# mpasha3/trips-py

Hardware: AMD Instinct MI355X
Metric: krylov_iters_per_sec (higher is better)
Workload: dtype f32

## Files before the change

### include/trk.h

```cpp
#ifndef TRK_H
#define TRK_H

#include <stdint.h>

#ifdef __cplusplus
extern "C" {
#endif

#define TRK_OK 0
#define TRK_EINVAL (-1)
#define TRK_EHIP (-2)
#define TRK_ENOMEM (-3)
#define TRK_EUNSUPPORTED (-4)
#define TRK_ENCCL (-5)

#define TRK_SQRT_NUM 1
#define TRK_SQRT_DEN 2

typedef struct trk_op trk_op;
typedef void* trk_stream;
typedef struct trk_comm trk_comm;

int trk_version(void);
const char* trk_last_error(void);
// ... 171 lines not shown
                                  double beta0, double m_eff, double x1, double x2, double xatol, int maxfun);
int trk_host_worker_post_hess_fixed(trk_host_worker* w, const double* H, int64_t h_row_stride, int64_t h_col_stride, int k,
                                    double beta0, double lam);
int trk_host_worker_post_hess_dp(trk_host_worker* w, const double* H, int64_t h_row_stride, int64_t h_col_stride, int k,
                                 double beta0, const double* bproj, double target, double extra);
int trk_host_worker_collect_vec(trk_host_worker* w, double* lam_out, int* have_out, double* y, int k, double* resid_out);

int trk_cgls_iterate(trk_op* A, int k_first, int n_iters, float* p, float* r, float* t, float* w, float* X, int64_t x_ld,
                     int keep_history, const float* x_prev, const float* x_true, double* S, double* NP,
                     int np_capacity_blocks, int* n_np_inout, double* PG, double* PD, int pcap, int grouping,
                     trk_stream stream);
int trk_cgls_iterate_fused(trk_op* A, int k_first, int n_iters, float* P, int64_t p_ld, float* R, int64_t r_ld, float* t,
                           float* w, float* X, int64_t x_ld, int keep_history, const float* x_prev, const float* x_true,
                           double* S, double* PG, double* PD, int pcap, double* NP, int np_capacity_blocks,
                           int* n_g_inout, int* n_np_inout, trk_stream stream);

int trk_finalize_batched(const double* partials, int nblocks, int nvals, int batches, double* out, int out_stride,
                         trk_stream stream);

int trk_gemv_t(const float* V, int64_t ld, int k, int64_t n, const float* r, const float* w2, double* h_dev,
               trk_stream stream);
int trk_gemv_nt(const float* V, int64_t ld, int k, int64_t n, const double* h_dev, const float* w_in, float* w_out,
                double* g_dev, trk_stream stream);
int trk_gemv_t_x(const float* V, int64_t ld, int k, int64_t n, const float* r, const float* xrow, double* h, double* h_x,
                 trk_stream stream);
int trk_gemv_t2(const float* V, int64_t ld, int k, int64_t n, const float* r, const float* r2, double* h2k_dev,
                trk_stream stream);
int trk_cgs_coeffs(double* G_dev, int ldg, const double* h_dev, const double* g_new_dev, int k, int passes, double* c_dev,
                   trk_stream stream);
int trk_cgs_coeffs_rho(double* G_dev, int ldg, const double* h_dev, const double* g_new_dev, int k, int passes, double* c_dev,
// ... 83 lines not shown
```

### trips_py_amd/_lib.py

```python
import ctypes
import os
import shutil
import subprocess
import sys
from concurrent.futures import ThreadPoolExecutor

HERE = os.path.dirname(os.path.abspath(__file__))
CSRC = os.path.join(HERE, "csrc")
INCLUDE = os.path.join(os.path.dirname(HERE), "include")
LIB_PATH = os.path.join(CSRC, "libtrk.so")
SOURCES = ["core.hip", "vecops.hip", "blur2d.hip", "tvops.hip", "radon2d.hip", "spmv.hip", "fanbeam2d.hip", "projected.hip", "cgls_loop.hip", "comm.hip", "cgls_tiled.hip", "cgls_sharded.hip", "ref64.hip"]
HIPCC_FLAGS = ["-O3", "--offload-arch=gfx950", "-std=c++17", "-fPIC", "-I" + INCLUDE, "-I" + CSRC]


class TrkError(RuntimeError):
    pass


def _hipcc():
    exe = shutil.which("hipcc") or "/opt/rocm/bin/hipcc"
    if not os.path.exists(exe):
        raise TrkError("hipcc not found: cannot build libtrk.so (ROCm toolchain required)")
    return exe

# ... 173 lines not shown
                                   ctypes.POINTER(c_int), ctypes.POINTER(c_dbl)]),
    "trk_host_gcv_bidiag": (c_int, [c_f64p, c_f64p, c_int, c_dbl, c_dbl, c_dbl, c_dbl, c_dbl, c_int, ctypes.POINTER(c_dbl),
                                    ctypes.POINTER(c_dbl), ctypes.POINTER(c_int)]),
    "trk_cgls_iterate": (c_int, [c_op, c_int, c_int, c_f32p, c_f32p, c_f32p, c_f32p, c_f32p, c_i64, c_int, c_f32p, c_f32p,
                                 c_f64p, c_f64p, c_int, ctypes.POINTER(c_int), c_f64p, c_f64p, c_int, c_int, c_stream]),
    "trk_cgls_update_xr_src": (c_int, [c_i64, c_i64, c_f64p, c_int, c_f64p, c_int, c_f32p, c_f32p, c_f32p, c_f32p, c_f32p,
                                       c_f32p, c_f64p, c_f64p, c_int, ctypes.POINTER(c_int), c_stream]),
    "trk_cgls_update_grouping": (c_int, [c_i64]),
    "trk_cgls_r_update": (c_int, [c_i64, c_f64p, c_f64p, c_int, c_f32p, c_f32p, c_f64p, c_stream]),
    "trk_cgls_xp_update": (c_int, [c_i64, c_f64p, c_f64p, c_f64p, c_int, c_f32p, c_f32p, c_f32p, c_f32p, c_f32p, c_f64p, c_f64p,
                                   c_int, ctypes.POINTER(c_int), c_stream]),
    "trk_cgls_p_update": (c_int, [c_i64, c_f32p, c_f32p, c_f64p, c_int, c_f64p, c_f64p, c_stream]),
    "trk_cgls_iterate_fused": (c_int, [c_op, c_int, c_int, c_f32p, c_i64, c_f32p, c_i64, c_f32p, c_f32p, c_f32p, c_i64, c_int,
                                       c_f32p, c_f32p, c_f64p, c_f64p, c_f64p, c_int, c_f64p, c_int, ctypes.POINTER(c_int),
                                       ctypes.POINTER(c_int), c_stream]),
    "trk_cgls_tiled_caps": (c_int, [c_op, c_int, c_int, ctypes.POINTER(c_int)]),
    "trk_cgls_iterate_tiled": (c_int, [c_op, c_int, c_int, c_f32p, c_i64, c_f32p, c_i64, c_f32p, c_f32p, c_i64, c_int,
                                       c_f32p, c_f32p, c_f64p, c_f64p, c_f64p, c_int, c_f64p, c_int, ctypes.POINTER(c_int),
                                       ctypes.POINTER(c_int), c_stream]),
    "trk_cgls_iterate_tiled2": (c_int, [c_op, c_int, c_int, c_f32p, c_f32p, c_f32p, c_i64, c_f32p, c_f32p, c_i64, c_int,
                                        c_f32p, c_f32p, c_f64p, c_f64p, c_f64p, c_int, c_f64p, c_int, ctypes.POINTER(c_int),
                                        ctypes.POINTER(c_int), c_stream]),
    "trk_gemv_t": (c_int, [c_f32p, c_i64, c_int, c_i64, c_f32p, c_f32p, c_f64p, c_stream]),
    "trk_gemv_t_x": (c_int, [c_f32p, c_i64, c_int, c_i64, c_f32p, c_f32p, c_f64p, c_f64p, c_stream]),
    "trk_gemv_t2": (c_int, [c_f32p, c_i64, c_int, c_i64, c_f32p, c_f32p, c_f64p, c_stream]),
    "trk_gemv_tn": (c_int, [c_f32p, c_i64, c_int, c_i64, ctypes.POINTER(ctypes.c_void_p), c_int, c_f64p, c_stream]),
    "trk_gram_row_from_sweep": (c_int, [c_f64p, c_int, c_int, c_f64p, c_f64p, c_f64p, c_f64p, c_f64p, c_f64p, c_stream]),
    "trk_gram_tikhonov": (c_int, [c_f64p, c_int, c_f64p, c_int, c_f64p, c_int, c_dbl, c_f64p, c_int, c_int, c_f64p, c_stream]),
    "trk_hess_tikhonov": (c_int, [c_f64p, c_int, c_f64p, c_f64p, c_int, c_f64p, c_f64p, c_f64p, c_dbl, c_int, c_dbl, c_int, c_f64p,
                                  c_stream]),
# ... 113 lines not shown
```

### trips_py_amd/csrc/blur2d.hip

```cpp
#include "trk_internal.h"
#include <hip/hip_ext.h>

#include <cmath>
#include <cstdlib>
#include <type_traits>
#include <vector>

using namespace trk;

namespace {

constexpr int NT = 256;
constexpr int TW = 128;
constexpr int TH = 32;

typedef float f4 __attribute__((ext_vector_type(4)));

__host__ __device__ constexpr int rup4(int v) { return (v + 3) & ~3; }

__device__ __forceinline__ int reflect(int i, int n) {
  if ((unsigned)i < (unsigned)n) return i;
  const int p = 2 * n;
  i %= p;
  if (i < 0) i += p;
// ... 510 lines not shown
  if (trk_timer* t = op->timer)
    if ((op->timer_which == 2 || op->timer_which == tr) && t->used < t->cap) {
      ev0 = t->ev[2 * t->used];
      ev1 = t->ev[2 * t->used + 1];
      ++t->used;
    }
  switch (im->kh) {
    case 3: return launch_slide<3, 6>(im, tr, x1, 0, y, 0, 1, partials, spans_x, nbands, rpb, s, ev0, ev1, fzp);
    case 5: return launch_slide<5, 5>(im, tr, x1, 0, y, 0, 1, partials, spans_x, nbands, rpb, s, ev0, ev1, fzp);
    case 7: return launch_slide<7, 7>(im, tr, x1, 0, y, 0, 1, partials, spans_x, nbands, rpb, s, ev0, ev1, fzp);
    default:
      return launch_slide<9, 9>(im, tr, x1, 0, y, 0, 1, partials, spans_x, nbands, rpb, s, ev0, ev1, fzp);
  }
}

int blur_apply(trk_op* op, int tr, const float* x, int64_t ldx, float* y, int64_t ldy, int batch, double* sumsq,
               hipStream_t s) {
  auto* im = static_cast<BlurImpl*>(op->impl);
  double* part = nullptr;
  int nblk;
  const bool slide_ok = slide_shape_ok(im) && aligned16(x) && aligned16(y) &&
                        (batch == 1 || ((ldx & 3) == 0 && (ldy & 3) == 0));
  if (slide_ok) {
    int spans_x, nbands, rpb;
    const int Usel = (im->kh == 9) ? 9 : (im->kh == 7) ? 7 : (im->kh == 5) ? 5 : 6;
    slide_grid(im->nx, im->ny, batch, im->kh, Usel, &spans_x, &nbands, &rpb);
    nblk = spans_x * nbands;
    if (sumsq)
      if (int rc = scratch_doubles(s, (size_t)nblk * batch, &part)) return rc;
    hipEvent_t ev0 = nullptr, ev1 = nullptr;
// ... 171 lines not shown
    rc = upload(sf, &im->sep_dev[0]);
    if (!rc) rc = upload(st, &im->sep_dev[1]);
  }
  if (rc) {
    trk_op tmp{1, 0, 0, im, nullptr, nullptr, nullptr, 0};
    blur_destroy(&tmp);
    return rc;
  }
  const int64_t n = (int64_t)nx * ny;
  auto* op = new trk_op{1, n, n, im, blur_apply, blur_destroy, nullptr, 0};
  if (slide_shape_ok(im)) op->apply_fused = blur_apply_fused;
  if (slide_shape_ok(im)) op->apply_axpby_plain = blur_apply_axpby_plain;
  *out = op;
  return TRK_OK;
}
```

### trips_py_amd/csrc/cgls_loop.hip

```cpp
#include "trk_internal.h"

using namespace trk;

extern "C" {

int trk_cgls_update_grouping(int64_t n) {
  static const int env = getenv("TRK_CGLS_XP") ? atoi(getenv("TRK_CGLS_XP")) : -1;
  if (env >= 0) return env != 0;
  return n >= ((int64_t)8 << 20) ? 1 : 0;
}

int trk_cgls_iterate(trk_op* A, int k_first, int n_iters, float* p, float* r, float* t, float* w, float* X, int64_t x_ld,
                     int keep_history, const float* x_prev, const float* x_true, double* S, double* NP,
                     int np_capacity_blocks, int* n_np_inout, double* PG, double* PD, int pcap, int grouping,
                     trk_stream stream) {
  TRK_REQUIRE(A && p && r && t && w && X && x_prev && S && NP && n_np_inout, "trk_cgls_iterate: NULL argument");
  TRK_REQUIRE(k_first >= 1 && n_iters >= 0, "trk_cgls_iterate: need k_first >= 1, n_iters >= 0");
  const int64_t m = A->rows, n = A->cols;
  int n_np = *n_np_inout;
  const bool raw = PG && PD && pcap > 0 && A->apply_fused;
  const bool xp_form = (grouping < 0 ? trk_cgls_update_grouping(n) : grouping) == 1;
  for (int k = k_first; k < k_first + n_iters; ++k) {
    double* row = S + 5 * (int64_t)k;
    double *delta = row, *gamma = row + 1;
// ... 61 lines not shown
    if (rc) return rc;
    float* x_new = X + (int64_t)(keep_history ? (k - 1) : ((k - 1) & 1)) * x_ld;
    double* gpub = (k == 1) ? S : S + b - 4;
    rc = trk_cgls_x_update(n, PG, n_g, PD, n_d, x_prev, p_new, x_new, x_true, S + b, gpub,
                           NP + 3 * (int64_t)n_np * (k - 1), np_capacity_blocks, &n_np, stream);
    if (rc) return rc;
    rc = trk_op_apply_fused(A, 1, r_old, w, -1.0, gpub, 1, S + b, 1, r_new, t, PG, pcap, &n_g, stream);
    if (rc) return rc;
    x_prev = x_new;
  }
  *n_g_inout = n_g;
  *n_np_inout = n_np;
  return TRK_OK;
}

}
```

### trips_py_amd/csrc/trk_internal.h

```cpp
#pragma once
#include <hip/hip_runtime.h>
#include <stdint.h>
#include <stddef.h>
#include "trk.h"

namespace trk {

void set_error(const char* fmt, ...) __attribute__((format(printf, 1, 2)));
int fail(int code, const char* fmt, ...) __attribute__((format(printf, 2, 3)));

#define TRK_HIP(expr)                                                                         \
  do {                                                                                        \
    hipError_t e_ = (expr);                                                                   \
    if (e_ != hipSuccess) return ::trk::fail(TRK_EHIP, "%s -> %s (%s:%d)", #expr,             \
                                             hipGetErrorString(e_), __FILE__, __LINE__);      \
  } while (0)

#define TRK_REQUIRE(cond, ...)                                  \
  do {                                                          \
    if (!(cond)) return ::trk::fail(TRK_EINVAL, __VA_ARGS__);   \
  } while (0)

#define TRK_LAUNCH_CHECK() TRK_HIP(hipGetLastError())

// ... 220 lines not shown
  if (i + 256 < s.n) a4 += s.p[i + 256];
  if (i + 320 < s.n) a5 += s.p[i + 320];
  if (i + 384 < s.n) a6 += s.p[i + 384];
  double v = ((a0 + a1) + (a2 + a3)) + ((a4 + a5) + (a6 + a7));
  v = wave_sum(v);
  return __hiloint2double(__builtin_amdgcn_readfirstlane(__double2hiint(v)), __builtin_amdgcn_readfirstlane(__double2loint(v)));
}

inline int ceil_div(int64_t a, int64_t b) { return (int)((a + b - 1) / b); }

inline int stream_nontemporal(int64_t n) {
  static const int env = getenv("TRK_NT") ? atoi(getenv("TRK_NT")) : -1;
  static const int rev = (getenv("TRK_REV") && atoi(getenv("TRK_REV"))) ? 256 : 0;
  if (env >= 0) return env | rev;
  if (n >= kNontemporalLoadsMinFloats) return 51 | 192 | rev;
  return (n >= kNontemporalMinFloats ? (3 | 192) : 0) | rev;
}

inline bool aligned16(const void* p) { return (reinterpret_cast<uintptr_t>(p) & 15u) == 0; }

}

struct trk_timer {
  hipEvent_t* ev;
  int cap, used;
};

namespace trk {
struct TimerScope {
  trk_timer* t;
  hipStream_t s;
// ... 103 lines not shown
```

### trips_py_amd/engine.py

```python
import ctypes

import numpy as np
import torch

from . import _lib

SQRT_NUM = 1
SQRT_DEN = 2


class Coef:

    __slots__ = ("c", "num", "den", "flags", "_keep")

    def __init__(self, c=1.0, num=None, den=None, sqrt_num=False, sqrt_den=False):
        self.c = float(c)
        self.num = _ptr(num)
        self.den = _ptr(den)
        self.flags = (SQRT_NUM if sqrt_num else 0) | (SQRT_DEN if sqrt_den else 0)
        self._keep = (num, den)


_raw_stream = getattr(torch._C, "_cuda_getCurrentRawStream", None)
if _raw_stream is None:
# ... 439 lines not shown
                                       ctypes.byref(c), _ptr(PG), _ptr(PD), int(pcap), int(grouping), self.stream())
        _lib.check(rc, "trk_cgls_iterate")
        return c.value

    def cgls_iterate_fused(self, handle, k_first, n_iters, P, R, t, w, X, keep, x_prev, x_true, S, PG, PD, pcap, NP, np_cap,
                           n_g, n_np):
        cg, cn = ctypes.c_int(int(n_g)), ctypes.c_int(int(n_np))
        rc = self.lib.trk_cgls_iterate_fused(handle, int(k_first), int(n_iters), P.data_ptr(), P.stride(0), R.data_ptr(),
                                             R.stride(0), t.data_ptr(), w.data_ptr(), X.data_ptr(), X.stride(0),
                                             int(bool(keep)), x_prev.data_ptr(), None if x_true is None else x_true.data_ptr(),
                                             _ptr(S), _ptr(PG), _ptr(PD), int(pcap), _ptr(NP), int(np_cap), ctypes.byref(cg),
                                             ctypes.byref(cn), self.stream())
        _lib.check(rc, "trk_cgls_iterate_fused")
        return cg.value, cn.value

    def cgls_tiled_caps(self, handle, np_cap, pcap):
        can = ctypes.c_int(0)
        _lib.check(self.lib.trk_cgls_tiled_caps(handle, int(np_cap), int(pcap), ctypes.byref(can)), "trk_cgls_tiled_caps")
        return bool(can.value)

    def cgls_iterate_tiled(self, handle, k_first, n_iters, P, R, t, X, keep, x_prev, x_true, S, PG, PD, pcap, NP, np_cap,
                           n_g, n_np):
        cg, cn = ctypes.c_int(int(n_g)), ctypes.c_int(int(n_np))
        rc = self.lib.trk_cgls_iterate_tiled(handle, int(k_first), int(n_iters), P.data_ptr(), P.stride(0), R.data_ptr(),
                                             R.stride(0), t.data_ptr(), X.data_ptr(), X.stride(0), int(bool(keep)),
                                             x_prev.data_ptr(), None if x_true is None else x_true.data_ptr(), _ptr(S),
                                             _ptr(PG), _ptr(PD), int(pcap), _ptr(NP), int(np_cap), ctypes.byref(cg),
                                             ctypes.byref(cn), self.stream())
        _lib.check(rc, "trk_cgls_iterate_tiled")
        return cg.value, cn.value
# ... 237 lines not shown
```

### trips_py_amd/solvers/CGLS.py

```python
import numpy as np

from .._io import Formatter, History, as_operator
from ..engine import Coef


class _ShiftedRows:

    def __init__(self, t, shift):
        self.t, self.shift = t, int(shift)

    def data_ptr(self):
        return self.t.data_ptr() + self.shift * self.t.stride(0) * self.t.element_size()

    def stride(self, dim):
        return self.t.stride(dim)

    def row(self, j):
        return self.t[j + self.shift]


def _row_of(X, j, keep):
    if isinstance(X, _ShiftedRows):
        return X.row(j)
    return X[j] if keep else X[j & 1]
# ... 221 lines not shown
            rows = Sh[5:5 * (k + 1)].reshape(k, 5).copy()
            rows[:, 2:5] = Nh[:3 * k].reshape(k, 3)
            rows[k - 1, 1] = Nh[3 * k]
            self._rows = (k, Sh[0], rows)
        return self._rows[1], self._rows[2]

    def row(self, k):
        return self.rows()[1][k - 1]


class CGLSRunFused(CGLSRun):

    PCAP = 4096
    AUTO_MIN_N = 3 * 2 ** 20
    AUTO_MAX_N = 7 * 2 ** 20

    @classmethod
    def auto(cls, n):
        return cls.AUTO_MIN_N <= n <= cls.AUTO_MAX_N

    @staticmethod
    def usable(A, eng):
        return (getattr(eng, "is_native", False) and eng.world == 1 and hasattr(A, "_h") and A.shape[0] == A.shape[1]
                and eng.op_can_fuse(A._h) == 1)

    TILED_MAX_N = 1 << 20
    TILED_DEFAULT = 2

    @classmethod
    def tiled_usable(cls, A, eng):
        return (cls.usable(A, eng) and hasattr(eng, "cgls_tiled_caps") and A.shape[1] <= cls.TILED_MAX_N
                and eng.cgls_tiled_caps(A._h, 1024, cls.PCAP))

    def __init__(self, A, b, x0, max_iter, x_true=None, history=True, tiled=False):
        self.A = A = as_operator(A)
        self.eng = eng = A.engine
        m, n = A.shape
        self.tiled = int(tiled)
        self.max_iter = max_iter = int(max_iter)
        self.bv = eng.to_vec(b, m)
        self.xt = None if x_true is None else eng.to_vec(x_true, n)
        x_start = eng.to_vec(x0, n)
        self.hist = History(eng, history, max_iter, n, "CGLS xHistory")
        self.keep = self.hist.keeps_any
        self.X = self.hist.X
        self.R = eng.empty_basis(2, m)
        self.P = eng.empty_basis(2, n)
        if self.tiled != 2:
            self.P.zero_()
        self.t, self.w = eng.empty(n), eng.empty(m)
        self.S = S = eng.scalars(5 * (max_iter + 1))
        uninit = getattr(eng, "scalars_uninit", eng.scalars)
        self.PG = uninit(self.PCAP)
        self.PD = uninit(self.PCAP)
        self.NP = uninit(3 * 1024 * max_iter)
        self.dist = False
        self.k = 0
        self.n_g = self.n_np = 0
        A.apply(x_start, out=self.w)
        self.n_g = eng.op_apply_fused(A._h, True, self.bv, self.w, -1.0, None, 0, None, 0, self.R[0], self.t,
                                      self.PG.ref(0), self.PCAP)
        self.x_cur = x_start
        self._final = False

    def _step(self):
        eng, A, S = self.eng, self.A, self.S
        if self.tiled:
            x_new = self.hist.row(self.k)
            keep = self.hist.mode == "device"
            X = self.X if self.hist.mode != "stream" else _ShiftedRows(self.X, self.hist.slot(self.k) - self.k)
            self._tiled_call(self.k + 1, 1, X, keep or self.hist.mode == "stream")
            self.k += 1
            self.x_cur = x_new
            return
        self.k += 1
        k = self.k
        b = 5 * k
        p_old, p_new = self.P[(k - 1) & 1], self.P[k & 1]
        r_old, r_new = self.R[(k - 1) & 1], self.R[k & 1]
        gprev = S.ref(0) if k <= 2 else S.ref(5 * (k - 2) + 1)
        n_d = eng.op_apply_fused(A._h, False, self.t, p_old, 0.0 if k == 1 else 1.0, self.PG.ref(0), self.n_g, gprev, 1,
                                 p_new, self.w, self.PD.ref(0), self.PCAP)
        x_new = self.hist.row(k - 1)
        gpub = S.ref(0) if k == 1 else S.ref(b - 4)
        self.n_np = eng.cgls_x_update(self.PG.ref(0), self.n_g, self.PD.ref(0), n_d, self.x_cur, p_new, x_new, self.xt,
                                      S.ref(b), gpub, self.NP.ref(3 * self.n_np * (k - 1)), 1024)
        self.n_g = eng.op_apply_fused(A._h, True, r_old, self.w, -1.0, gpub, 1, S.ref(b), 1, r_new, self.t,
                                      self.PG.ref(0), self.PCAP)
        self.x_cur = x_new

    def _tiled_call(self, k_first, n, X, keep):
        eng = self.eng
        if self.tiled == 2:
            self.n_g, self.n_np = eng.cgls_iterate_tiled2(self.A._h, k_first, n, self.P[0], self.w, self.R, self.t, X, keep,
                                                          self.x_cur, self.xt, self.S.ref(0), self.PG.ref(0), self.PD.ref(0),
                                                          self.PCAP, self.NP.ref(0), 1024, self.n_g, self.n_np)
        else:
            self.n_g, self.n_np = eng.cgls_iterate_tiled(self.A._h, k_first, n, self.P, self.R, self.t, X, keep, self.x_cur, self.xt,
                                                         self.S.ref(0), self.PG.ref(0), self.PD.ref(0), self.PCAP, self.NP.ref(0),
                                                         1024, self.n_g, self.n_np)

    def run(self, n_steps):
        n_steps = min(int(n_steps), self.max_iter - self.k)
        if n_steps <= 0:
            return
        def call(k_first, n, X, keep):
            if self.tiled:
                self._tiled_call(k_first, n, X, keep)
            else:
                self.n_g, self.n_np = self.eng.cgls_iterate_fused(self.A._h, k_first, n, self.P, self.R, self.t, self.w,
                                                                  X, keep, self.x_cur, self.xt, self.S.ref(0),
                                                                  self.PG.ref(0), self.PD.ref(0), self.PCAP, self.NP.ref(0), 1024,
                                                                  self.n_g, self.n_np)
            self.x_cur = _row_of(X, k_first + n - 2, keep)
        self._run_c_loop(n_steps, call)

    def _finish(self):
        if self.k == 0 or self._final == self.k:
            return
        eng, S, k = self.eng, self.S, self.k
        eng.finalize_batched(self.NP.ref(0), self.n_np, 3, k, S.ref(7), 5)
        eng.finalize_batched(self.PG.ref(0), self.n_g, 1, 1, S.ref(5 * k + 1), 1)
        self._final = k
# ... 62 lines not shown
```

Before: 7306.

## Add lagged CGLS path fusing blur apply with vector updates in ring kernels

Result: faster. 7482, median of 6 (+2.4%).

```diff
diff --git a/include/trk.h b/include/trk.h
--- a/include/trk.h
+++ b/include/trk.h
@@ -209,6 +209,17 @@
                            float* w, float* X, int64_t x_ld, int keep_history, const float* x_prev, const float* x_true,
                            double* S, double* PG, double* PD, int pcap, double* NP, int np_capacity_blocks,
                            int* n_g_inout, int* n_np_inout, trk_stream stream);
+int trk_cgls_lagged_k1(trk_op* A, const float* t, const float* p_old, double sign, const double* gamma_part, int n_g,
+                       const double* gamma_prev, double* pub_gamma, float* p_new, float* w, double* PD, int pcap, int* n_d,
+                       const float* x, float* x_new, const float* x_true, const double* delta_prev, double* NP, int np_cap,
+                       trk_stream st);
+int trk_cgls_lagged_k2(trk_op* A, const float* r_old, const float* w, const double* gamma, const double* delta_part, int n_d,
+                       double* pub_delta, float* r_new, float* t, double* PG, int pcap, int* n_g, const float* p, const float* x,
+                       float* x_new, const float* x_true, double* NP, int np_cap, trk_stream st);
+int trk_cgls_iterate_lagged(trk_op* A, int k_first, int n_iters, float* P, int64_t p_ld, float* R, int64_t r_ld, float* t,
+                            float* w, float* X, int64_t x_ld, int keep_history, const float* x_prev, const float* x_true,
+                            double* S, double* PG, double* PD, int pcap, double* NP, int np_capacity_blocks, int* n_g_inout,
+                            int* n_np_inout, trk_stream stream);
 
 int trk_finalize_batched(const double* partials, int nblocks, int nvals, int batches, double* out, int out_stride,
                          trk_stream stream);
diff --git a/trips_py_amd/_lib.py b/trips_py_amd/_lib.py
--- a/trips_py_amd/_lib.py
+++ b/trips_py_amd/_lib.py
@@ -211,6 +211,13 @@
     "trk_cgls_iterate_fused": (c_int, [c_op, c_int, c_int, c_f32p, c_i64, c_f32p, c_i64, c_f32p, c_f32p, c_f32p, c_i64, c_int,
                                        c_f32p, c_f32p, c_f64p, c_f64p, c_f64p, c_int, c_f64p, c_int, ctypes.POINTER(c_int),
                                        ctypes.POINTER(c_int), c_stream]),
+    "trk_cgls_lagged_k1": (c_int, [c_op, c_f32p, c_f32p, c_dbl, c_f64p, c_int, c_f64p, c_f64p, c_f32p, c_f32p, c_f64p, c_int,
+                                   ctypes.POINTER(c_int), c_f32p, c_f32p, c_f32p, c_f64p, c_f64p, c_int, c_stream]),
+    "trk_cgls_lagged_k2": (c_int, [c_op, c_f32p, c_f32p, c_f64p, c_f64p, c_int, c_f64p, c_f32p, c_f32p, c_f64p, c_int,
+                                   ctypes.POINTER(c_int), c_f32p, c_f32p, c_f32p, c_f32p, c_f64p, c_int, c_stream]),
+    "trk_cgls_iterate_lagged": (c_int, [c_op, c_int, c_int, c_f32p, c_i64, c_f32p, c_i64, c_f32p, c_f32p, c_f32p, c_i64, c_int,
+                                        c_f32p, c_f32p, c_f64p, c_f64p, c_f64p, c_int, c_f64p, c_int, ctypes.POINTER(c_int),
+                                        ctypes.POINTER(c_int), c_stream]),
     "trk_cgls_tiled_caps": (c_int, [c_op, c_int, c_int, ctypes.POINTER(c_int)]),
     "trk_cgls_iterate_tiled": (c_int, [c_op, c_int, c_int, c_f32p, c_i64, c_f32p, c_i64, c_f32p, c_f32p, c_i64, c_int,
                                        c_f32p, c_f32p, c_f64p, c_f64p, c_f64p, c_int, c_f64p, c_int, ctypes.POINTER(c_int),
diff --git a/trips_py_amd/csrc/blur2d.hip b/trips_py_amd/csrc/blur2d.hip
--- a/trips_py_amd/csrc/blur2d.hip
+++ b/trips_py_amd/csrc/blur2d.hip
@@ -1,4 +1,5 @@
 #include "trk_internal.h"
+#include "cgls_ring.h"
 #include <hip/hip_ext.h>
 
 #include <cmath>
@@ -548,6 +549,72 @@
   }
 }
 
+inline int ring_grid(int nx, int ny, int kh, int U, int cap, int* spans_x, int* nbands, int* rows_per_band) {
+  const int sx = ceil_div(ny, ring::SPAN);
+  const int64_t most = std::min<int64_t>(4 * (int64_t)cu_count(), cap);
+  int rows = U;
+  while (rows - (kh - 1) < kh + 1) rows += U;
+  for (;; rows += U) {
+    const int r = rows - (kh - 1);
+    if ((int64_t)sx * ceil_div(nx, r) <= most || r >= nx) break;
+  }
+  *spans_x = sx;
+  *rows_per_band = rows - (kh - 1);
+  *nbands = ceil_div(nx, *rows_per_band);
+  return sx * *nbands;
+}
+
+template <int K, int D, int RIDE, bool XT>
+void ring_launch(const ring::Args& a, int nblk, hipStream_t s, hipEvent_t ev0, hipEvent_t ev1) {
+  hipExtLaunchKernelGGL((ring::k_cgls_ring<K, D, RIDE, XT>), dim3(nblk), dim3(64), D * ring::ring_slot_bytes(RIDE, XT), s, ev0, ev1,
+                        0, a);
+}
+template <int K, int D>
+void ring_launch_k(const ring::Args& a, int ride, int nblk, hipStream_t s, hipEvent_t ev0, hipEvent_t ev1) {
+  const bool xt = ride && a.x_true;
+  if (ride == 0) ring_launch<K, D, 0, false>(a, nblk, s, ev0, ev1);
+  else if (ride == 1) { if (xt) ring_launch<K, D, 1, true>(a, nblk, s, ev0, ev1); else ring_launch<K, D, 1, false>(a, nblk, s, ev0, ev1); }
+  else { if (xt) ring_launch<K, D, 2, true>(a, nblk, s, ev0, ev1); else ring_launch<K, D, 2, false>(a, nblk, s, ev0, ev1); }
+}
+
+int blur_cgls_ring(trk_op* op, int tr, ring::Args a, int ride, int cap, int* n_partials, hipStream_t s) {
+  if (!op || op->kind != 1) return fail(TRK_EUNSUPPORTED, "lagged CGLS: needs a blur2d handle");
+  auto* im = static_cast<BlurImpl*>(op->impl);
+  const bool al = aligned16(a.a) && aligned16(a.b) && aligned16(a.comb) && aligned16(a.y) &&
+                  (!ride || (aligned16(a.x) && aligned16(a.x_new) && (!a.x_true || aligned16(a.x_true)) && (ride != 2 || aligned16(a.p))));
+  if (!slide_shape_ok(im) || !al)
+    return fail(TRK_EUNSUPPORTED, "lagged CGLS: needs a separable odd PSF <= 9x9, ny %% 4 == 0, 16-byte aligned vectors");
+  if (a.comb == a.a || a.comb == a.b) return fail(TRK_EINVAL, "lagged CGLS: the combined operand must not alias an input");
+  if (ride && (a.x_new == a.x)) return fail(TRK_EINVAL, "lagged CGLS: x_new must not alias x");
+  const int U = (im->kh == 3) ? 6 : im->kh;
+  int nblk = ring_grid(im->nx, im->ny, im->kh, U, cap, &a.spans_x, &a.nbands, &a.rows_per_band);
+  if (nblk > cap) return fail(TRK_EINVAL, "lagged CGLS: partial buffers hold %d blocks, %d needed", cap, nblk);
+  *n_partials = nblk;
+  a.nx = im->nx;
+  a.ny = im->ny;
+  const int nts = stream_nontemporal((int64_t)im->nx * im->ny);
+  a.nt_y = (nts & 1) && !(tr == 1 && (nts & 512));
+  a.nt_x = (nts >> 1) & 1;
+  a.nt_comb = tr == 1 ? (nts >> 2) & 1 : (nts >> 3) & 1;
+  a.nt_ld = (nts >> 10) & 3;
+  a.wts = im->sep_dev[tr];
+  hipEvent_t ev0 = nullptr, ev1 = nullptr;
+  if (trk_timer* t = op->timer)
+    if ((op->timer_which == 2 || op->timer_which == tr) && t->used < t->cap) {
+      ev0 = t->ev[2 * t->used];
+      ev1 = t->ev[2 * t->used + 1];
+      ++t->used;
+    }
+  switch (im->kh) {
+    case 3: ring_launch_k<3, 6>(a, ride, nblk, s, ev0, ev1); break;
+    case 5: ring_launch_k<5, 5>(a, ride, nblk, s, ev0, ev1); break;
+    case 7: ring_launch_k<7, 7>(a, ride, nblk, s, ev0, ev1); break;
+    default: ring_launch_k<9, 9>(a, ride, nblk, s, ev0, ev1); break;
+  }
+  TRK_LAUNCH_CHECK();
+  return TRK_OK;
+}
+
 int blur_apply(trk_op* op, int tr, const float* x, int64_t ldx, float* y, int64_t ldy, int batch, double* sumsq,
                hipStream_t s) {
   auto* im = static_cast<BlurImpl*>(op->impl);
@@ -749,3 +816,56 @@
   *out = op;
   return TRK_OK;
 }
+
+extern "C" int trk_cgls_lagged_k1(trk_op* A, const float* t, const float* p_old, double sign, const double* gamma_part, int n_g,
+                                  const double* gamma_prev, double* pub_gamma, float* p_new, float* w, double* PD, int pcap,
+                                  int* n_d, const float* x, float* x_new, const float* x_true, const double* delta_prev,
+                                  double* NP, int np_cap, trk_stream st) {
+  TRK_REQUIRE(A && t && p_old && gamma_part && n_g >= 1 && gamma_prev && p_new && w && PD && n_d, "trk_cgls_lagged_k1: NULL argument");
+  TRK_REQUIRE(!x || (x_new && delta_prev && NP), "trk_cgls_lagged_k1: the x update needs x_new, delta_prev and NP");
+  ring::Args a{};
+  a.a = t;
+  a.b = p_old;
+  a.comb = p_new;
+  a.y = w;
+  a.part = PD;
+  a.sign = sign;
+  a.num = ScalarSrc{gamma_part, n_g};
+  a.den = ScalarSrc{gamma_prev, 1};
+  a.pub_num = pub_gamma;
+  a.pub_den = nullptr;
+  a.x = x;
+  a.x_new = x_new;
+  a.x_true = x ? x_true : nullptr;
+  a.rg = ScalarSrc{gamma_prev, 1};
+  a.rd = ScalarSrc{delta_prev, 1};
+  a.np = NP;
+  return blur_cgls_ring(A, 0, a, x ? 1 : 0, x ? std::min(pcap, np_cap) : pcap, n_d, (hipStream_t)st);
+}
+
+extern "C" int trk_cgls_lagged_k2(trk_op* A, const float* r_old, const float* w, const double* gamma, const double* delta_part,
+                                  int n_d, double* pub_delta, float* r_new, float* t, double* PG, int pcap, int* n_g,
+                                  const float* p, const float* x, float* x_new, const float* x_true, double* NP, int np_cap,
+                                  trk_stream st) {
+  TRK_REQUIRE(A && r_old && w && gamma && delta_part && n_d >= 1 && r_new && t && PG && n_g, "trk_cgls_lagged_k2: NULL argument");
+  TRK_REQUIRE(!p || (x && x_new && NP), "trk_cgls_lagged_k2: the x update needs x, x_new and NP");
+  ring::Args a{};
+  a.a = r_old;
+  a.b = w;
+  a.comb = r_new;
+  a.y = t;
+  a.part = PG;
+  a.sign = -1.0;
+  a.num = ScalarSrc{gamma, 1};
+  a.den = ScalarSrc{delta_part, n_d};
+  a.pub_num = nullptr;
+  a.pub_den = pub_delta;
+  a.p = p;
+  a.x = x;
+  a.x_new = x_new;
+  a.x_true = p ? x_true : nullptr;
+  a.rg = a.num;
+  a.rd = a.den;
+  a.np = NP;
+  return blur_cgls_ring(A, 1, a, p ? 2 : 0, p ? std::min(pcap, np_cap) : pcap, n_g, (hipStream_t)st);
+}
diff --git a/trips_py_amd/csrc/cgls_loop.hip b/trips_py_amd/csrc/cgls_loop.hip
--- a/trips_py_amd/csrc/cgls_loop.hip
+++ b/trips_py_amd/csrc/cgls_loop.hip
@@ -99,4 +99,45 @@
   return TRK_OK;
 }
 
+int trk_cgls_iterate_lagged(trk_op* A, int k_first, int n_iters, float* P, int64_t p_ld, float* R, int64_t r_ld, float* t,
+                            float* w, float* X, int64_t x_ld, int keep_history, const float* x_prev, const float* x_true,
+                            double* S, double* PG, double* PD, int pcap, double* NP, int np_capacity_blocks, int* n_g_inout,
+                            int* n_np_inout, trk_stream stream) {
+  TRK_REQUIRE(A && P && R && t && w && X && x_prev && S && PG && PD && NP && n_g_inout && n_np_inout,
+              "trk_cgls_iterate_lagged: NULL argument");
+  TRK_REQUIRE(k_first >= 1 && n_iters >= 0, "trk_cgls_iterate_lagged: need k_first >= 1, n_iters >= 0");
+  int n_g = *n_g_inout, n_np = *n_np_inout, n_d = 0;
+  auto slot = [&](int j) { return X + (int64_t)(keep_history ? (j - 1) : ((j - 1) & 1)) * x_ld; };
+  const float* xc = x_prev;
+  const int k_last = k_first + n_iters - 1;
+  for (int k = k_first; k <= k_last; ++k) {
+    float *p_old = P + (int64_t)((k - 1) & 1) * p_ld, *p_new = P + (int64_t)(k & 1) * p_ld;
+    float *r_old = R + (int64_t)((k - 1) & 1) * r_ld, *r_new = R + (int64_t)(k & 1) * r_ld;
+    const double* gprev = (k <= 2) ? S : S + 5 * (int64_t)(k - 2) + 1;
+    double* gpub = (k == 1) ? S : S + 5 * (int64_t)(k - 1) + 1;
+    const bool ride1 = k > k_first;
+    int nb = 0;
+    int rc = trk_cgls_lagged_k1(A, t, p_old, k == 1 ? 0.0 : 1.0, PG, n_g, gprev, gpub, p_new, w, PD, pcap, &n_d,
+                                ride1 ? xc : nullptr, ride1 ? slot(k - 1) : nullptr, x_true, S + 5 * (int64_t)(k - 1),
+                                ride1 ? NP + 3 * (int64_t)n_d * (k - 2) : nullptr, np_capacity_blocks, stream);
+    if (rc) return rc;
+    if (ride1) {
+      if (n_np != 0 && n_np != n_d) return fail(TRK_EINVAL, "trk_cgls_iterate_lagged: norm partials were laid out for %d blocks", n_np);
+      n_np = n_d;
+      xc = slot(k - 1);
+    }
+    const bool ride2 = k == k_last;
+    if (ride2 && n_np != 0 && n_np != n_d)
+      return fail(TRK_EINVAL, "trk_cgls_iterate_lagged: norm partials were laid out for %d blocks", n_np);
+    rc = trk_cgls_lagged_k2(A, r_old, w, gpub, PD, n_d, S + 5 * (int64_t)k, r_new, t, PG, pcap, &nb, ride2 ? p_new : nullptr,
+                            xc, slot(k), x_true, ride2 ? NP + 3 * (int64_t)n_d * (k - 1) : nullptr, np_capacity_blocks, stream);
+    if (rc) return rc;
+    n_g = nb;
+    if (ride2) n_np = n_d;
+  }
+  *n_g_inout = n_g;
+  *n_np_inout = n_np;
+  return TRK_OK;
 }
+
+}
diff --git a/trips_py_amd/csrc/cgls_ring.h b/trips_py_amd/csrc/cgls_ring.h
--- /dev/null
+++ b/trips_py_amd/csrc/cgls_ring.h
@@ -0,0 +1,318 @@
+#pragma once
+#include "trk_internal.h"
+
+namespace trk {
+namespace ring {
+
+typedef float f4 __attribute__((ext_vector_type(4)));
+typedef float f2 __attribute__((ext_vector_type(2)));
+typedef unsigned int u4 __attribute__((ext_vector_type(4)));
+typedef int i4 __attribute__((ext_vector_type(4)));
+
+constexpr int SPAN = 256;
+constexpr unsigned OOB = 0x80000000u;
+
+__host__ __device__ constexpr int gcd_c(int a, int b) { return b == 0 ? a : gcd_c(b, a % b); }
+__host__ __device__ constexpr int lcm_c(int a, int b) { return a / gcd_c(a, b) * b; }
+__host__ __device__ constexpr int pmod(int a, int m) { return ((a % m) + m) % m; }
+__host__ __device__ constexpr int cmin(int a, int b) { return a < b ? a : b; }
+
+__device__ __forceinline__ int reflect(int i, int n) {
+  if ((unsigned)i < (unsigned)n) return i;
+  const int p = 2 * n;
+  i %= p;
+  if (i < 0) i += p;
+  return (i >= n) ? (p - 1 - i) : i;
+}
+
+__device__ __forceinline__ i4 rsrc(const void* p, unsigned bytes) {
+  const uint64_t a = (uint64_t)p;
+  return (i4){(int)(unsigned)a, (int)((a >> 32) & 0xffffu), (int)bytes, 0x00020000};
+}
+__device__ __forceinline__ void dma_buf(i4 rs, unsigned voff, unsigned lds, bool nt) {
+  unsigned keep;
+  if (nt)
+    asm volatile("s_mov_b32 %0, m0\n\ts_mov_b32 m0, %3\n\ts_nop 0\n\tbuffer_load_dwordx4 %1, %2, 0 offen nt lds\n\ts_mov_b32 m0, %0"
+                 : "=&s"(keep) : "v"(voff), "s"(rs), "s"(lds) : "memory");
+  else
+    asm volatile("s_mov_b32 %0, m0\n\ts_mov_b32 m0, %3\n\ts_nop 0\n\tbuffer_load_dwordx4 %1, %2, 0 offen lds\n\ts_mov_b32 m0, %0"
+                 : "=&s"(keep) : "v"(voff), "s"(rs), "s"(lds) : "memory");
+}
+__device__ __forceinline__ void dma_glb(const float* g, unsigned lds, bool nt) {
+  unsigned keep;
+  if (nt)
+    asm volatile("s_mov_b32 %0, m0\n\ts_mov_b32 m0, %2\n\ts_nop 0\n\tglobal_load_lds_dwordx4 %1, off nt\n\ts_mov_b32 m0, %0"
+                 : "=&s"(keep) : "v"(g), "s"(lds) : "memory");
+  else
+    asm volatile("s_mov_b32 %0, m0\n\ts_mov_b32 m0, %2\n\ts_nop 0\n\tglobal_load_lds_dwordx4 %1, off\n\ts_mov_b32 m0, %0"
+                 : "=&s"(keep) : "v"(g), "s"(lds) : "memory");
+}
+__device__ __forceinline__ f4 lds128(unsigned a) {
+  f4 v;
+  asm volatile("ds_read_b128 %0, %1" : "=v"(v) : "v"(a) : "memory");
+  return v;
+}
+__device__ __forceinline__ void st128(f4 v, __amdgpu_buffer_rsrc_t rs, unsigned off, bool nt) {
+  if (nt) __builtin_amdgcn_raw_buffer_store_b128(__builtin_bit_cast(u4, v), rs, off, 0, 2);
+  else __builtin_amdgcn_raw_buffer_store_b128(__builtin_bit_cast(u4, v), rs, off, 0, 0);
+}
+__device__ __forceinline__ void lds_wait() { asm volatile("s_waitcnt lgkmcnt(0)" ::: "memory"); }
+__device__ __forceinline__ void tie(f4& v) { asm volatile("" : "+v"(v)); }
+
+#define TRK_VM_CASE(N) \
+  case N: asm volatile("s_waitcnt vmcnt(" #N ")" ::: "memory"); break;
+__device__ __forceinline__ void wait_vm(int n) {
+  switch (n < 63 ? n : 63) {
+    TRK_VM_CASE(0) TRK_VM_CASE(1) TRK_VM_CASE(2) TRK_VM_CASE(3) TRK_VM_CASE(4) TRK_VM_CASE(5) TRK_VM_CASE(6) TRK_VM_CASE(7)
+    TRK_VM_CASE(8) TRK_VM_CASE(9) TRK_VM_CASE(10) TRK_VM_CASE(11) TRK_VM_CASE(12) TRK_VM_CASE(13) TRK_VM_CASE(14) TRK_VM_CASE(15)
+    TRK_VM_CASE(16) TRK_VM_CASE(17) TRK_VM_CASE(18) TRK_VM_CASE(19) TRK_VM_CASE(20) TRK_VM_CASE(21) TRK_VM_CASE(22) TRK_VM_CASE(23)
+    TRK_VM_CASE(24) TRK_VM_CASE(25) TRK_VM_CASE(26) TRK_VM_CASE(27) TRK_VM_CASE(28) TRK_VM_CASE(29) TRK_VM_CASE(30) TRK_VM_CASE(31)
+    TRK_VM_CASE(32) TRK_VM_CASE(33) TRK_VM_CASE(34) TRK_VM_CASE(35) TRK_VM_CASE(36) TRK_VM_CASE(37) TRK_VM_CASE(38) TRK_VM_CASE(39)
+    TRK_VM_CASE(40) TRK_VM_CASE(41) TRK_VM_CASE(42) TRK_VM_CASE(43) TRK_VM_CASE(44) TRK_VM_CASE(45) TRK_VM_CASE(46) TRK_VM_CASE(47)
+    TRK_VM_CASE(48) TRK_VM_CASE(49) TRK_VM_CASE(50) TRK_VM_CASE(51) TRK_VM_CASE(52) TRK_VM_CASE(53) TRK_VM_CASE(54) TRK_VM_CASE(55)
+    TRK_VM_CASE(56) TRK_VM_CASE(57) TRK_VM_CASE(58) TRK_VM_CASE(59) TRK_VM_CASE(60) TRK_VM_CASE(61) TRK_VM_CASE(62)
+    default: asm volatile("s_waitcnt vmcnt(63)" ::: "memory"); break;
+  }
+}
+#undef TRK_VM_CASE
+
+struct Args {
+  const float* a;
+  const float* b;
+  float* comb;
+  float* y;
+  double* part;
+  double sign;
+  ScalarSrc num, den;
+  double* pub_num;
+  double* pub_den;
+  const float* p;
+  const float* x;
+  float* x_new;
+  const float* x_true;
+  ScalarSrc rg, rd;
+  double* np;
+  int nx, ny, spans_x, nbands, rows_per_band;
+  int nt_y, nt_comb, nt_x, nt_ld;
+  const float* wts;
+};
+
+__host__ __device__ constexpr int ring_ops(int ride, bool xt) { return 2 + (ride == 2 ? 1 : 0) + (ride ? 1 + (xt ? 1 : 0) : 0); }
+__host__ __device__ constexpr int ring_slot_bytes(int ride, bool xt) { return ring_ops(ride, xt) * 1024 + 64; }
+
+template <int KH, int D, int RIDE, bool XT>
+__global__ __launch_bounds__(64) void k_cgls_ring(Args g) {
+  constexpr int KW = KH;
+  constexpr int T = KH - 1 - KH / 2;
+  constexpr int Lh = KW - 1 - KW / 2;
+  constexpr int OFFC = 4 - Lh;
+  constexpr int U = lcm_c(KH, D);
+  constexpr int NC = ring_ops(RIDE, XT);
+  constexpr int NI = NC + 1;
+  constexpr int NS = 2 + (RIDE ? 1 : 0);
+  constexpr int SLOT = ring_slot_bytes(RIDE, XT);
+  constexpr int OP = (RIDE == 2) ? 2 : -1, OX = (RIDE == 2) ? 3 : 2, OXT = OX + 1;
+  static_assert(U % D == 0, "ring index must repeat with the unrolled block");
+  static_assert(Lh <= 4 && KW / 2 <= 4, "halos of at most one 4-column group");
+  extern __shared__ f4 ring_smem[];
+
+  const int nx = g.nx, ny = g.ny, spans_x = g.spans_x;
+  int band, span;
+  {
+    const int id = blockIdx.x, total = g.nbands * spans_x;
+    const int xcd = id & 7, local = id >> 3;
+    const int t = xcd * (total >> 3) + min(xcd, total & 7) + local;
+    band = t / spans_x;
+    span = t - band * spans_x;
+  }
+  const int i_begin = band * g.rows_per_band;
+  const int i_end = (i_begin + g.rows_per_band < nx) ? i_begin + g.rows_per_band : nx;
+  const int lane = threadIdx.x;
+  const int c0 = span * SPAN + 4 * lane;
+  const bool active = c0 < ny;
+  const int cc = active ? c0 : ny - 4;
+  const bool ledge = (c0 == 0), redge = (c0 + 4 == ny);
+  const bool edge_span = (span == 0) || ((span + 1) * SPAN >= ny);
+
+  const unsigned img_bytes = (unsigned)nx * (unsigned)ny * 4u;
+  const i4 ra = rsrc(g.a, img_bytes), rb = rsrc(g.b, img_bytes);
+  const i4 rp = rsrc(RIDE == 2 ? g.p : g.a, img_bytes), rx = rsrc(RIDE ? g.x : g.a, img_bytes);
+  const i4 rxt = rsrc(XT ? g.x_true : g.a, img_bytes);
+  const auto rcomb = __builtin_amdgcn_make_buffer_rsrc((void*)g.comb, 0, img_bytes, 0x00020000);
+  const auto rout = __builtin_amdgcn_make_buffer_rsrc((void*)g.y, 0, img_bytes, 0x00020000);
+  const auto rxn = __builtin_amdgcn_make_buffer_rsrc((void*)(RIDE ? g.x_new : g.y), 0, img_bytes, 0x00020000);
+
+  float cb = 0.f, step = 0.f;
+  {
+    const bool need_num = g.sign != 0.0 || g.pub_num != nullptr;
+    const bool need_den = g.sign != 0.0 || g.pub_den != nullptr;
+    const double vn = need_num ? scalar_from_wave(g.num, lane) : 0.0;
+    const double vd = need_den ? scalar_from_wave(g.den, lane) : 0.0;
+    if (g.sign != 0.0) cb = (float)(g.sign * vn / vd);
+    if (blockIdx.x == 0 && lane == 0) {
+      if (g.pub_num) *g.pub_num = vn;
+      if (g.pub_den) *g.pub_den = vd;
+    }
+    if (RIDE) step = (float)(scalar_from_wave(g.rg, lane) / scalar_from_wave(g.rd, lane));
+  }
+  const bool up = (band & 1) != 0;
+  float wr[KW], wc[KH];
+#pragma unroll
+  for (int b = 0; b < KW; ++b) wr[b] = g.wts[b];
+#pragma unroll
+  for (int a = 0; a < KH; ++a) wc[a] = up ? g.wts[KW + KH - 1 - a] : g.wts[KW + a];
+  asm volatile("s_waitcnt vmcnt(0) lgkmcnt(0)" ::: "memory");
+
+  const int band_rows = i_end - i_begin;
+  const int total = ((band_rows + KH - 1 + U - 1) / U) * U;
+  const unsigned rowbytes = (unsigned)ny * 4u;
+  const int dir = up ? -1 : 1;
+  const int first = up ? (i_end - 1 + KH / 2) : (i_begin - T);
+  const int last = first + dir * (total - 1);
+  const bool interior = (first >= 0) && (first < nx) && (last >= 0) && (last < nx);
+  const int ofirst = up ? (i_end - 1) : i_begin;
+  const unsigned vc = (unsigned)cc * 4u, vst = (unsigned)c0 * 4u;
+
+  const int hcl = span * SPAN >= 4 ? span * SPAN - 4 : 0;
+  const int hcr = (span * SPAN + SPAN + 4 <= ny) ? span * SPAN + SPAN : ny - 4;
+  const float* hsrc = ((lane & 2) ? g.b : g.a) + ((lane & 1) ? hcr : hcl);
+
+  const unsigned lds0 = (unsigned)(size_t)(__attribute__((address_space(3))) f4*)ring_smem;
+  const unsigned hbase = NC * 1024;
+  const unsigned oC = 16u * lane;
+  const unsigned oL = lane > 0 ? oC - 16u : hbase, oR = lane < 63 ? oC + 16u : hbase + 16u;
+  const unsigned obL = lane > 0 ? 1024u + oC - 16u : hbase + 32u, obR = lane < 63 ? 1024u + oC + 16u : hbase + 48u;
+
+  const bool ntl = (g.nt_ld & 1) != 0, nth = (g.nt_ld & 2) != 0;
+  auto issue = [&](int t, int slot) {
+    const int graw = first + dir * t;
+    const int gi = interior ? graw : reflect(graw, nx);
+    const unsigned ro = (unsigned)gi * rowbytes;
+    const unsigned lb = lds0 + (unsigned)slot * SLOT;
+    dma_buf(ra, vc + ro, lb, ntl);
+    dma_buf(rb, vc + ro, lb + 1024, ntl);
+    if (RIDE) {
+      const bool owned = graw >= i_begin && graw < i_end;
+      const unsigned po = owned ? vc + ro : OOB;
+      if (RIDE == 2) dma_buf(rp, po, lb + OP * 1024, ntl);
+      dma_buf(rx, po, lb + OX * 1024, ntl);
+      if (XT) dma_buf(rxt, po, lb + OXT * 1024, ntl);
+    }
+    if (lane < 4) dma_glb(hsrc + (int64_t)gi * ny, lb + hbase, nth);
+  };
+#pragma unroll
+  for (int d = 0; d < D; ++d) issue(d, d);
+
+  f2 acc[KH][2];
+  double ss = 0.0, s0 = 0.0, s1 = 0.0, s2 = 0.0;
+  float qacc = 0.f;
+  const bool nt_y = g.nt_y != 0, nt_x = g.nt_x != 0, nt_c = g.nt_comb != 0;
+
+  auto block = [&](int t0, auto first_tag, auto last_tag) {
+    constexpr bool FIRST = decltype(first_tag)::value, LAST = decltype(last_tag)::value;
+#pragma unroll
+    for (int u = 0; u < U; ++u) {
+      const int t = t0 + u;
+      const int slot = u % D;
+      const int rows_after = LAST ? cmin(D - 1, U - 1 - u) : D - 1;
+      const int steps_after = FIRST ? cmin(u, D) : D;
+      wait_vm(rows_after * NI + steps_after * NS);
+      const unsigned sb = lds0 + (unsigned)slot * SLOT;
+      f4 aL = lds128(sb + oL), aC = lds128(sb + oC), aR = lds128(sb + oR);
+      f4 bL = lds128(sb + obL), bC = lds128(sb + 1024 + oC), bR = lds128(sb + obR);
+      f4 pv = bC, xv = bC, xtv = bC;
+      if (RIDE == 2) pv = lds128(sb + OP * 1024 + oC);
+      if (RIDE) xv = lds128(sb + OX * 1024 + oC);
+      if (RIDE && XT) xtv = lds128(sb + OXT * 1024 + oC);
+      lds_wait();
+      tie(aL); tie(aC); tie(aR); tie(bL); tie(bC); tie(bR);
+      if (RIDE == 2) tie(pv);
+      if (RIDE) tie(xv);
+      if (RIDE && XT) tie(xtv);
+      if (RIDE == 1) pv = bC;
+      if (!LAST || u + D < U) issue(t + D, slot);
+
+      const int graw = first + dir * t;
+      const bool owned = graw >= i_begin && graw < i_end;
+      f4 Lv = aL, Cv = aC, Rv = aR;
+      Lv = Lv + cb * bL;
+      Cv = Cv + cb * bC;
+      Rv = Rv + cb * bR;
+      st128(Cv, rcomb, (owned && active) ? vst + (unsigned)graw * rowbytes : OOB, nt_c);
+      if (RIDE) {
+        const float d0 = step * pv[0], d1 = step * pv[1], d2 = step * pv[2], d3 = step * pv[3];
+        const float xn0 = xv[0] + d0, xn1 = xv[1] + d1, xn2 = xv[2] + d2, xn3 = xv[3] + d3;
+        const f4 xn = (f4){xn0, xn1, xn2, xn3};
+        st128(xn, rxn, (owned && active) ? vst + (unsigned)graw * rowbytes : OOB, nt_x);
+        if (owned && active) {
+          s0 += (double)xn0 * xn0 + (double)xn1 * xn1 + (double)xn2 * xn2 + (double)xn3 * xn3;
+          s1 += (double)d0 * d0 + (double)d1 * d1 + (double)d2 * d2 + (double)d3 * d3;
+          if (XT) {
+            const double e0 = (double)xn0 - xtv[0], e1 = (double)xn1 - xtv[1], e2 = (double)xn2 - xtv[2], e3 = (double)xn3 - xtv[3];
+            s2 += e0 * e0 + e1 * e1 + e2 * e2 + e3 * e3;
+          }
+        }
+      }
+      if (edge_span) {
+        const f4 rev = (f4){Cv[3], Cv[2], Cv[1], Cv[0]};
+        if (ledge) Lv = rev;
+        if (redge) Rv = rev;
+      }
+      const float v[12] = {Lv[0], Lv[1], Lv[2], Lv[3], Cv[0], Cv[1], Cv[2], Cv[3], Rv[0], Rv[1], Rv[2], Rv[3]};
+      float h0 = 0.f, h1 = 0.f, h2 = 0.f, h3 = 0.f;
+#pragma unroll
+      for (int b = 0; b < KW; ++b) {
+        h0 = fmaf(wr[b], v[OFFC + b], h0);
+        h1 = fmaf(wr[b], v[OFFC + b + 1], h1);
+        h2 = fmaf(wr[b], v[OFFC + b + 2], h2);
+        h3 = fmaf(wr[b], v[OFFC + b + 3], h3);
+      }
+      const f2 hlo = {h0, h1}, hhi = {h2, h3};
+#pragma unroll
+      for (int a = 0; a < KH; ++a) {
+        const int k = pmod(u - a, KH);
+        if (a == 0) {
+          acc[k][0] = wc[0] * hlo;
+          acc[k][1] = wc[0] * hhi;
+        } else {
+          acc[k][0] = wc[a] * hlo + acc[k][0];
+          acc[k][1] = wc[a] * hhi + acc[k][1];
+        }
+      }
+      const int o = t - (KH - 1);
+      const bool ovalid = o >= 0 && o < band_rows;
+      const int kd = pmod(u - (KH - 1), KH);
+      const f4 out = (f4){acc[kd][0][0], acc[kd][0][1], acc[kd][1][0], acc[kd][1][1]};
+      st128(out, rout, (ovalid && active) ? vst + (unsigned)(ofirst + dir * o) * rowbytes : OOB, nt_y);
+      if (ovalid && active) qacc = fmaf(out[0], out[0], fmaf(out[1], out[1], fmaf(out[2], out[2], fmaf(out[3], out[3], qacc))));
+      if ((u & 3) == 3) {
+        ss += (double)qacc;
+        qacc = 0.f;
+      }
+    }
+  };
+  if (total == U) {
+    block(0, std::true_type{}, std::true_type{});
+  } else {
+    block(0, std::true_type{}, std::false_type{});
+    int t0 = U;
+    for (; t0 + U < total; t0 += U) block(t0, std::false_type{}, std::false_type{});
+    block(t0, std::false_type{}, std::true_type{});
+  }
+  ss += (double)qacc;
+  ss = wave_sum(ss);
+  if (lane == 0) g.part[blockIdx.x] = ss;
+  if (RIDE) {
+    s0 = wave_sum(s0);
+    s1 = wave_sum(s1);
+    if (XT) s2 = wave_sum(s2);
+    if (lane == 0) {
+      g.np[blockIdx.x * 3 + 0] = s0;
+      g.np[blockIdx.x * 3 + 1] = s1;
+      g.np[blockIdx.x * 3 + 2] = XT ? s2 : 0.0;
+    }
+  }
+}
+
+}
+}
diff --git a/trips_py_amd/csrc/trk_internal.h b/trips_py_amd/csrc/trk_internal.h
--- a/trips_py_amd/csrc/trk_internal.h
+++ b/trips_py_amd/csrc/trk_internal.h
@@ -258,7 +258,7 @@
   static const int rev = (getenv("TRK_REV") && atoi(getenv("TRK_REV"))) ? 256 : 0;
   if (env >= 0) return env | rev;
   if (n >= kNontemporalLoadsMinFloats) return 51 | 192 | rev;
-  return (n >= kNontemporalMinFloats ? (3 | 192) : 0) | rev;
+  return (n >= kNontemporalMinFloats ? (3 | 192 | 1024) : 0) | rev;
 }
 
 inline bool aligned16(const void* p) { return (reinterpret_cast<uintptr_t>(p) & 15u) == 0; }
diff --git a/trips_py_amd/engine.py b/trips_py_amd/engine.py
--- a/trips_py_amd/engine.py
+++ b/trips_py_amd/engine.py
@@ -477,6 +477,40 @@
         _lib.check(rc, "trk_cgls_iterate_fused")
         return cg.value, cn.value
 
+    def cgls_iterate_lagged(self, handle, k_first, n_iters, P, R, t, w, X, keep, x_prev, x_true, S, PG, PD, pcap, NP, np_cap,
+                            n_g, n_np):
+        cg, cn = ctypes.c_int(int(n_g)), ctypes.c_int(int(n_np))
+        rc = self.lib.trk_cgls_iterate_lagged(handle, int(k_first), int(n_iters), P.data_ptr(), P.stride(0), R.data_ptr(),
+                                              R.stride(0), t.data_ptr(), w.data_ptr(), X.data_ptr(), X.stride(0),
+                                              int(bool(keep)), x_prev.data_ptr(), None if x_true is None else x_true.data_ptr(),
+                                              _ptr(S), _ptr(PG), _ptr(PD), int(pcap), _ptr(NP), int(np_cap), ctypes.byref(cg),
+                                              ctypes.byref(cn), self.stream())
+        _lib.check(rc, "trk_cgls_iterate_lagged")
+        return cg.value, cn.value
+
+    def cgls_lagged_k1(self, handle, t, p_old, sign, gamma_part, n_g, gamma_prev, pub_gamma, p_new, w, PD, pcap,
+                       x=None, x_new=None, x_true=None, delta_prev=None, NP=None, np_cap=0):
+        n = ctypes.c_int(0)
+        rc = self.lib.trk_cgls_lagged_k1(handle, t.data_ptr(), p_old.data_ptr(), float(sign), _ptr(gamma_part), int(n_g),
+                                         _ptr(gamma_prev), _ptr(pub_gamma), p_new.data_ptr(), w.data_ptr(), _ptr(PD), int(pcap),
+                                         ctypes.byref(n), None if x is None else x.data_ptr(),
+                                         None if x_new is None else x_new.data_ptr(),
+                                         None if x_true is None else x_true.data_ptr(), _ptr(delta_prev), _ptr(NP), int(np_cap),
+                                         self.stream())
+        _lib.check(rc, "trk_cgls_lagged_k1")
+        return n.value
+
+    def cgls_lagged_k2(self, handle, r_old, w, gamma, delta_part, n_d, pub_delta, r_new, t, PG, pcap,
+                       p=None, x=None, x_new=None, x_true=None, NP=None, np_cap=0):
+        n = ctypes.c_int(0)
+        rc = self.lib.trk_cgls_lagged_k2(handle, r_old.data_ptr(), w.data_ptr(), _ptr(gamma), _ptr(delta_part), int(n_d),
+                                         _ptr(pub_delta), r_new.data_ptr(), t.data_ptr(), _ptr(PG), int(pcap), ctypes.byref(n),
+                                         None if p is None else p.data_ptr(), None if x is None else x.data_ptr(),
+                                         None if x_new is None else x_new.data_ptr(),
+                                         None if x_true is None else x_true.data_ptr(), _ptr(NP), int(np_cap), self.stream())
+        _lib.check(rc, "trk_cgls_lagged_k2")
+        return n.value
+
     def cgls_tiled_caps(self, handle, np_cap, pcap):
         can = ctypes.c_int(0)
         _lib.check(self.lib.trk_cgls_tiled_caps(handle, int(np_cap), int(pcap), ctypes.byref(can)), "trk_cgls_tiled_caps")
diff --git a/trips_py_amd/solvers/CGLS.py b/trips_py_amd/solvers/CGLS.py
--- a/trips_py_amd/solvers/CGLS.py
+++ b/trips_py_amd/solvers/CGLS.py
@@ -259,10 +259,16 @@
     PCAP = 4096
     AUTO_MIN_N = 3 * 2 ** 20
     AUTO_MAX_N = 7 * 2 ** 20
+    LAGGED_MIN_N = 11 << 20
+    LAGGED_MAX_N = 20 << 20
 
     @classmethod
     def auto(cls, n):
-        return cls.AUTO_MIN_N <= n <= cls.AUTO_MAX_N
+        return cls.AUTO_MIN_N <= n <= cls.AUTO_MAX_N or cls.lagged_auto(n)
+
+    @classmethod
+    def lagged_auto(cls, n):
+        return cls.LAGGED_MIN_N <= n < cls.LAGGED_MAX_N
 
     @staticmethod
     def usable(A, eng):
@@ -277,11 +283,13 @@
         return (cls.usable(A, eng) and hasattr(eng, "cgls_tiled_caps") and A.shape[1] <= cls.TILED_MAX_N
                 and eng.cgls_tiled_caps(A._h, 1024, cls.PCAP))
 
-    def __init__(self, A, b, x0, max_iter, x_true=None, history=True, tiled=False):
+    def __init__(self, A, b, x0, max_iter, x_true=None, history=True, tiled=False, lagged=None):
         self.A = A = as_operator(A)
         self.eng = eng = A.engine
         m, n = A.shape
         self.tiled = int(tiled)
+        want = self.lagged_auto(n) if lagged is None else bool(lagged)
+        self.lagged = want and self.tiled == 0 and hasattr(eng, "cgls_iterate_lagged")
         self.max_iter = max_iter = int(max_iter)
         self.bv = eng.to_vec(b, m)
         self.xt = None if x_true is None else eng.to_vec(x_true, n)
@@ -310,11 +318,14 @@
 
     def _step(self):
         eng, A, S = self.eng, self.A, self.S
-        if self.tiled:
+        if self.tiled or self.lagged:
             x_new = self.hist.row(self.k)
             keep = self.hist.mode == "device"
             X = self.X if self.hist.mode != "stream" else _ShiftedRows(self.X, self.hist.slot(self.k) - self.k)
-            self._tiled_call(self.k + 1, 1, X, keep or self.hist.mode == "stream")
+            if self.tiled:
+                self._tiled_call(self.k + 1, 1, X, keep or self.hist.mode == "stream")
+            else:
+                self._lagged_call(self.k + 1, 1, X, keep or self.hist.mode == "stream")
             self.k += 1
             self.x_cur = x_new
             return
@@ -334,6 +345,11 @@
                                       self.PG.ref(0), self.PCAP)
         self.x_cur = x_new
 
+    def _lagged_call(self, k_first, n, X, keep):
+        self.n_g, self.n_np = self.eng.cgls_iterate_lagged(self.A._h, k_first, n, self.P, self.R, self.t, self.w, X, keep, self.x_cur,
+                                                           self.xt, self.S.ref(0), self.PG.ref(0), self.PD.ref(0), self.PCAP,
+                                                           self.NP.ref(0), 1024, self.n_g, self.n_np)
+
     def _tiled_call(self, k_first, n, X, keep):
         eng = self.eng
         if self.tiled == 2:
@@ -352,6 +368,8 @@
         def call(k_first, n, X, keep):
             if self.tiled:
                 self._tiled_call(k_first, n, X, keep)
+            elif self.lagged:
+                self._lagged_call(k_first, n, X, keep)
             else:
                 self.n_g, self.n_np = self.eng.cgls_iterate_fused(self.A._h, k_first, n, self.P, self.R, self.t, self.w,
                                                                   X, keep, self.x_cur, self.xt, self.S.ref(0),
```
